# asharakeh/pod_compare

Hardware: AMD Instinct MI355X
Metric: images/sec (BayesOD+MC-dropout, 1280x720) (higher is better)
Workload: dtype f32 (convolutions: every fp32 product from 2-way f16 splits of the power-of-two-scaled fp32 operands, 3 partial products, fp32 accumulate; closer to fp64 than the fp32 MFMA: profiles/r05_f16_split_numerics.txt)

## Files before the change

include/pod_mi355x.h:

```cpp
#ifndef POD_MI355X_H
#define POD_MI355X_H

#include <stddef.h>
#include <stdint.h>

#ifdef __cplusplus
extern "C" {
#endif

#define POD_ABI_VERSION 18
#define POD_MAX_LEVELS 8
#define POD_MAX_CLASSES 16
#define POD_MAX_RUNS 64
#define POD_MAX_TOPK 2048
#define POD_MAX_PROP_SAMPLES 1024
#define POD_MAX_CLS_SAMPLES 64
#define POD_MAX_CANDIDATES 8192
#define POD_MAX_DETECTIONS 128
#define POD_COCO_MAX_IOU 16
#define POD_COCO_MAX_REC 128
#define POD_COCO_MAX_AREA 4
#define POD_COCO_MAX_MAXDET 4
#define POD_COCO_MAX_KEEP 128
#define POD_COCO_LDS_GT 64
// ... 57 lines not shown

int pod_level_topk(const PodConfig* cfg, const PodLevel* levels, uint64_t* cand_keys,
                   int32_t* cand_count, uint64_t* sel_keys, int32_t* sel_count,
                   uint64_t* cat_keys, int32_t* cat_level, int32_t* n_total, pod_stream_t stream);

int pod_gather_candidates(const PodConfig* cfg, const PodLevel* levels, const float* anchors,
                          const uint64_t* cat_keys, const int32_t* cat_level, const int32_t* n_total,
                          int32_t* cand_count, const float* probs_dense,
                          int32_t* cand_anchor_idx, int32_t* cand_level, float* cand_score, int32_t* cand_class,
                          float* cand_probs, float* cand_delta, float* cand_reg_var, float* cand_anchor,
                          float* cand_run_delta ,
                          pod_stream_t stream);

int pod_decode_cov(const PodConfig* cfg, const PodLevel* levels, const int32_t* n_total, int32_t n_capacity,
                   const float* cand_delta, const float* cand_reg_var, const float* cand_anchor,
                   const float* cand_run_delta, const int32_t* cand_anchor_idx, const int32_t* cand_level,
                   const float* eps_prop, int32_t n_replay,
                   float* boxes, float* cov, pod_stream_t stream);

int pod_gather_decode(const PodConfig* cfg, const PodLevel* levels, const float* anchors, const uint64_t* cat_keys,
                      const int32_t* cat_level, const int32_t* n_total, int32_t* cand_count, const float* probs_dense,
                      int32_t* cand_anchor_idx, int32_t* cand_level, float* cand_score,
                      int32_t* cand_class, float* cand_probs, float* cand_delta, float* cand_reg_var, float* cand_anchor,
                      float* cand_run_delta, float* boxes, float* cov, pod_stream_t stream);

size_t pod_nms_scratch_bytes(int32_t n_capacity);
int pod_nms_cluster(const PodConfig* cfg, const int32_t* n_total, int32_t n_capacity,
                    const float* boxes, const float* scores, const int32_t* classes,
                    int32_t* keep, int32_t* n_keep, void* scratch, pod_stream_t stream);

int pod_bayes_fuse(const PodConfig* cfg, const int32_t* n_total, const int32_t* keep, const int32_t* n_keep,
                   const float* boxes, const float* cov, const float* scores, const int32_t* classes,
                   const float* probs, int32_t box_mode, int32_t cls_mode,
                   float* out_boxes, float* out_cov, float* out_scores, int32_t* out_classes, float* out_probs,
                   pod_stream_t stream);

int pod_anchor_stats_merge(const PodConfig* cfg, const int32_t* n_total, const int32_t* keep, const int32_t* n_keep,
                           const float* boxes, const float* cov, const int32_t* classes, const float* probs,
                           float* out_boxes, float* out_cov, float* out_scores, int32_t* out_classes, float* out_probs,
                           pod_stream_t stream);

int pod_ensemble_append(const PodConfig* cfg, const int32_t* keep, const int32_t* n_keep, const float* boxes, const float* cov,
                        const int32_t* classes, const float* probs, int32_t capacity,
                        float* dst_boxes, float* dst_cov, int32_t* dst_classes, float* dst_probs, int32_t* total,
                        pod_stream_t stream);
int pod_ensemble_merge(const PodConfig* cfg, const int32_t* m_total, int32_t capacity, const float* boxes, const float* cov,
                       const int32_t* classes, const float* probs, int32_t* seeds, int32_t* n_seeds,
                       float* out_boxes, float* out_cov, float* out_scores, int32_t* out_classes, float* out_probs,
                       pod_stream_t stream);

int pod_finalize(const PodConfig* cfg, const int32_t* keep, const int32_t* n_rows,
                 const float* boxes, const float* cov, const float* scores, const int32_t* classes,
                 const float* probs, float scale_x, float scale_y, float out_h, float out_w,
                 float* det_boxes, float* det_cov, float* det_scores, int32_t* det_classes, float* det_probs,
                 float* records, int32_t* n_det, pod_stream_t stream);

typedef struct PodDetections {
    float* boxes;  float* cov;  float* scores;  int32_t* classes;  float* probs;  float* records;  int32_t* n_det;
} PodDetections;

int pod_relu_dropout(float* x, int64_t n, float p, uint64_t seed, uint64_t offset, pod_stream_t stream);

int pod_bias_act(float* x, const float* bias, const float* residual, const float* res_bias, int64_t n, int32_t C,
                 int64_t HW, int32_t relu, float p, uint64_t seed, uint64_t offset, pod_stream_t stream);

int pod_bias_act_to_nchw(const float* src, float* dst, const float* bias, int64_t N, int32_t C, int64_t HW, int32_t relu,
                         float p, uint64_t seed, uint64_t offset, pod_stream_t stream);
int pod_bias_act_to_nhwc(const float* src, float* dst, const float* bias, int64_t N, int32_t C, int64_t HW, int32_t relu,
                         pod_stream_t stream);

int pod_expand_dropout(const float* src, float* dst, int64_t n, int32_t copies, float p, uint64_t seed, uint64_t offset,
                       const uint64_t* epoch, pod_stream_t stream);

int pod_wino_filter_transform(const float* weight, float* U, int32_t K, int32_t C, pod_stream_t stream);
int pod_wino_conv3x3(const float* in, float* out, const float* U, const float* bias, const int32_t* blocks, int32_t n_blocks,
                     int32_t C, int32_t K, int32_t k_planes, int32_t relu, float p, uint64_t seed, uint64_t offset,
                     const uint64_t* epoch, pod_stream_t stream);

#define POD_AMAX_SLOTS 16
#define POD_AMAX_STRIDE 32
#define POD_AMAX_FLOATS (POD_AMAX_SLOTS * POD_AMAX_STRIDE)
int pod_absmax(const float* x, int64_t n, float* amax, pod_stream_t stream);

typedef struct PodConvSet {
    const float* in;
    float* out;
    const void* Us;
    const float* bias;
    const float* in_amax;
    float* out_amax;
    uint64_t offset;
    int32_t first_block;
    int32_t replicas;
    int32_t k_planes;
    int32_t reserved;
} PodConvSet;
typedef struct PodWinoConv {
    const int32_t* blocks;
    int32_t n_blocks, n_sets;
    int32_t C, K, relu;
    float p;
    uint64_t seed;
    const uint64_t* epoch;
    int32_t n_splits;
    int32_t reserved;
    int64_t split_stride;
    const int32_t* live_blocks;
    PodConvSet sets[4];
} PodWinoConv;
int64_t pod_wino_filter_split_bytes(int32_t K, int32_t C);
int pod_wino_filter_transform_split(const float* weight, void* Us, int32_t K, int32_t C, pod_stream_t stream);
int pod_wino_conv3x3_split(const PodWinoConv* conv, pod_stream_t stream);

#define POD_SPARSE_LIVE_HEAD 4
#define POD_SPARSE_LIVE_STRIDE 12
int pod_sparse_reach(const PodConfig* cfg, const PodLevel* levels, const uint64_t* cat_keys, const int32_t* cat_level, const int32_t* n_total,
                     uint8_t* reach, uint8_t* scratch, pod_stream_t stream);
int pod_sparse_live_blocks(const PodConfig* cfg, const PodLevel* levels, const int32_t* records, const int32_t* rec_level, int32_t n_records,
                           const uint8_t* reach, int32_t max_reach, int32_t in_reach, int32_t* live, pod_stream_t stream);
int pod_wino_reduce(const float* partials, int32_t n_splits, int64_t split_stride, const float* bias, float* planes, int64_t HW,
                    int32_t K, int32_t k_real, int32_t relu, float* out_amax, pod_stream_t stream);

int pod_stem7x7_filter_split(const float* weight, void* Ws, pod_stream_t stream);
int pod_stem7x7_split(const void* x, int32_t x_is_u8, int32_t H_img, int32_t W_img, const float* mean, const float* stddev, float* y, const void* Ws,
                      const float* bias, int32_t H, int32_t W, int32_t relu, const float* in_amax, float* out_amax, pod_stream_t stream);
int pod_maxpool3x3s2_cl(const float* x, float* y, int32_t H, int32_t W, int32_t C, pod_stream_t stream);
int pod_im2col3x3s2_cl(const float* x, float* y, int32_t H, int32_t W, int32_t C, int32_t relu, pod_stream_t stream);

int pod_match_groundtruth(const float* det_boxes, const float* det_probs, const int32_t* det_off, const int32_t* det_img,
                          int32_t n_det, const float* gt_boxes, const int32_t* gt_off, const int32_t* gt_img, int32_t n_gt,
                          int32_t num_classes, float iou_min, float iou_correct, int32_t* gt_fn, int32_t* gt_match_count,
                          int32_t* gt_match_idx, float* gt_match_iou, int32_t* det_fp, pod_stream_t stream);

int pod_reg_nll(const float* means, const float* covs, const float* gt, int32_t n, float* nll, pod_stream_t stream);

typedef struct PodCocoParams {
    int32_t n_iou, n_rec, n_area, n_maxdet;
    int32_t n_cat;
    int32_t reserved;
    double iou_thrs[POD_COCO_MAX_IOU];
    double rec_thrs[POD_COCO_MAX_REC];
    double area_rng[2 * POD_COCO_MAX_AREA];
    int32_t max_dets[POD_COCO_MAX_MAXDET];
} PodCocoParams;

size_t pod_coco_eval_scratch_bytes(int32_t n_keep, int32_t n_gt);
int pod_coco_eval_images(const PodCocoParams* prm, const int64_t* pairs, int32_t n_pairs, const double* dt_boxes,
                         const double* dt_score, const double* gt_boxes, const double* gt_area, const int32_t* gt_crowd,
                         const int64_t* gt_id, void* scratch, double* kept_score, uint64_t* kept_match, uint64_t* kept_ignore,
                         int32_t* kept_rank, int32_t* npig, pod_stream_t stream);

size_t pod_coco_accumulate_workspace_bytes(int64_t n_kept);
int pod_coco_accumulate(const PodCocoParams* prm, const int64_t* cat_off, int32_t max_seg, int64_t n_kept, const double* kept_score,
                        const uint64_t* kept_match, const uint64_t* kept_ignore, const int32_t* kept_rank, const int32_t* npig,
                        void* workspace, double* precision, double* recall, double* scores, pod_stream_t stream);


int pod_calib_keys(const float* cls_probs, int32_t k1, const float* cov, const int32_t* gt_class, int32_t n_matched, int32_t n,
                   float* cls_entropy, float* reg_entropy, int32_t* det_class, int32_t* class_count, pod_stream_t stream);

int pod_calib_reg_counts(const float* means, const float* cov, const float* gt, const int32_t* det_class, int32_t n_matched,
                         const float* edges, int32_t n_edges, int32_t* counts, pod_stream_t stream);

size_t pod_calib_min_uncertainty_workspace_bytes(int32_t n, int64_t n_pos);
int pod_calib_min_uncertainty(const float* cls_entropy, const float* reg_entropy, const int32_t* det_class, int32_t n, int32_t n_tp,
                              const int32_t* class_off, const int64_t* seg_off, const int32_t* seg_class, int32_t n_seg, int32_t max_seg,
// ... 167 lines not shown
```

pod_compare_amd/csrc/pod_device.h:

```cpp
#pragma once

#include <hip/hip_runtime.h>
#include <stdint.h>

#include <mutex>

#include "../../include/pod_mi355x.h"

#define POD_WAVE 64
#define POD_EPS_MAX 4.9f

#define POD_CHECK_LAUNCH()                                  \
    do {                                                    \
        if (hipGetLastError() != hipSuccess) return POD_E_LAUNCH; \
    } while (0)

template <auto Kernel>
static int pod_lds_opt_in(int bytes) {
    static std::once_flag once[64];
    static hipError_t attr[64];
    int dev = 0;
    if (hipGetDevice(&dev) != hipSuccess || dev < 0 || dev >= 64) return POD_E_LAUNCH;
    std::call_once(once[dev], [dev, bytes] {
        attr[dev] = hipFuncSetAttribute(reinterpret_cast<const void*>(Kernel), hipFuncAttributeMaxDynamicSharedMemorySize, bytes);
    });
    return attr[dev] == hipSuccess ? POD_OK : POD_E_LAUNCH;
}

template <typename... P>
static inline bool pod_aligned(unsigned bytes, const P*... p) {
    return ((... | reinterpret_cast<uintptr_t>(p)) & (bytes - 1u)) == 0;
}
static inline unsigned pod_grid_stride_blocks(int64_t n4, int64_t cap) {
    const int64_t blocks = (n4 + 255) / 256;
    return (unsigned)(blocks < 1 ? 1 : blocks > cap ? cap : blocks);
}

#ifdef POD_TRACE
static __device__ long long g_pod_trace[4096 * 8];
#define POD_STAMP(wg, k)                                                                         \
    do {                                                                                         \
        if ((threadIdx.x & 63) == 0 && threadIdx.x < 64 && (wg) < 4096) g_pod_trace[(wg) * 8 + (k)] = wall_clock64(); \
    } while (0)
#else
#define POD_STAMP(wg, k)
#endif

namespace pod {

struct u32x4 {
    uint32_t x, y, z, w;
};

__device__ __forceinline__ u32x4 philox4x32_10(u32x4 c, uint32_t k0, uint32_t k1) {
    constexpr uint32_t M0 = 0xD2511F53u, M1 = 0xCD9E8D57u, W0 = 0x9E3779B9u, W1 = 0xBB67AE85u;
#pragma unroll
    for (int r = 0; r < 10; ++r) {
        const uint64_t p0 = (uint64_t)M0 * c.x;
        const uint64_t p1 = (uint64_t)M1 * c.z;
        u32x4 n;
        n.x = (uint32_t)(p1 >> 32) ^ c.y ^ k0;
        n.y = (uint32_t)p1;
        n.z = (uint32_t)(p0 >> 32) ^ c.w ^ k1;
        n.w = (uint32_t)p0;
        c = n;
        k0 += W0;
        k1 += W1;
    }
    return c;
}

typedef float f32x4 __attribute__((ext_vector_type(4)));

constexpr uint32_t STREAM_DROPOUT = 0x64726f70u;
#define POD_DROPOUT_THRESH16(p) ((uint32_t)((double)(p) * 65536.0))

__device__ __forceinline__ uint64_t dropout_key(uint64_t seed, const uint64_t* epoch) {
    return epoch ? seed ^ (*epoch * 0x9E3779B97F4A7C15ull) : seed;
}
__device__ __forceinline__ void dropout_words(uint64_t base, uint64_t g, uint32_t c2, uint64_t seed, uint32_t& w0, uint32_t& w1) {
    const uint64_t ctr = base + (g >> 1);
    const u32x4 r = philox4x32_10(u32x4{(uint32_t)ctr, (uint32_t)(ctr >> 32), c2, STREAM_DROPOUT}, (uint32_t)seed, (uint32_t)(seed >> 32));
    w0 = (g & 1) ? r.z : r.x;
    w1 = (g & 1) ? r.w : r.y;
}
template <typename V4>
__device__ __forceinline__ void dropout_mask4(V4& v, uint32_t w0, uint32_t w1, uint32_t thresh, float scale) {
    v.x = (w0 & 0xFFFFu) >= thresh ? v.x * scale : 0.f;
    v.y = (w0 >> 16) >= thresh ? v.y * scale : 0.f;
    v.z = (w1 & 0xFFFFu) >= thresh ? v.z * scale : 0.f;
    v.w = (w1 >> 16) >= thresh ? v.w * scale : 0.f;
}
__device__ __forceinline__ bool dropout_tail_keep(uint64_t base, int64_t n4, uint32_t t, uint64_t seed, uint32_t thresh) {
    const uint64_t ctr = base + (uint64_t)n4 + t;
    const u32x4 r = philox4x32_10(u32x4{(uint32_t)ctr, (uint32_t)(ctr >> 32), 1u, STREAM_DROPOUT}, (uint32_t)seed, (uint32_t)(seed >> 32));
    return (r.x & 0xFFFFu) >= thresh;
}

__device__ __forceinline__ void box_muller16(uint32_t w, float& n0, float& n1) {
    const float u1 = ((float)(w & 0xFFFFu) + 0.5f) * 1.52587890625e-05f;
    const float u2 = ((float)(w >> 16) + 0.5f) * 1.52587890625e-05f;
    const float rad = __builtin_amdgcn_sqrtf(-1.3862943611198906f * __builtin_amdgcn_logf(u1));
    n0 = rad * __builtin_amdgcn_cosf(u2);
    n1 = rad * __builtin_amdgcn_sinf(u2);
}

struct f32x8n {
    float v[8];
};

constexpr uint32_t STREAM_CLS = 0x636c7300u;
constexpr uint32_t STREAM_BOX = 0x626f7800u;

__device__ __forceinline__ f32x8n philox_normals8(uint64_t seed, uint32_t c0, uint32_t c1, uint32_t c2, uint32_t stream) {
    const u32x4 r = philox4x32_10(u32x4{c0, c1, c2, stream}, (uint32_t)seed, (uint32_t)(seed >> 32));
    f32x8n o;
    box_muller16(r.x, o.v[0], o.v[1]);
    box_muller16(r.y, o.v[2], o.v[3]);
    box_muller16(r.z, o.v[4], o.v[5]);
    box_muller16(r.w, o.v[6], o.v[7]);
    return o;
}


__device__ __forceinline__ float sigmoid_ref(float x) { return __fdiv_rn(1.0f, 1.0f + expf(-x)); }
__device__ __forceinline__ float sigmoid_fast(float x) {
    return __builtin_amdgcn_rcpf(1.0f + __builtin_amdgcn_exp2f(-1.4426950408889634f * x));
}

struct Box {
    float x1, y1, x2, y2;
};
#define POD_SCALE_CLAMP 4.135166556742356f

__device__ __forceinline__ Box decode_box(float d0, float d1, float d2, float d3, const Box& a, const float* wts) {
    const float w = a.x2 - a.x1;
    const float h = a.y2 - a.y1;
    const float cx = a.x1 + 0.5f * w;
    const float cy = a.y1 + 0.5f * h;
    const bool unit = wts[0] == 1.0f && wts[1] == 1.0f && wts[2] == 1.0f && wts[3] == 1.0f;
    const float dx = unit ? d0 : __fdiv_rn(d0, wts[0]);
    const float dy = unit ? d1 : __fdiv_rn(d1, wts[1]);
    float dw = unit ? d2 : __fdiv_rn(d2, wts[2]);
    float dh = unit ? d3 : __fdiv_rn(d3, wts[3]);
    dw = fminf(dw, POD_SCALE_CLAMP);
    dh = fminf(dh, POD_SCALE_CLAMP);
// ... 57 lines not shown
```

pod_compare_amd/csrc/pod_wino.h:

```cpp
#pragma once
#include "pod_experiments.h"
#include "pod_split_gemm.h"

namespace pod {

constexpr int WINO_U_FLOATS = 24 * 2 * 64 * 4;
constexpr int WINO_SB_FLOATS = 384 * 32;
constexpr int WINO_LDS_BYTES = 4 * 32 * 4 * 65 * 4;

#ifdef POD_TRACE
static __device__ long long g_wino_trace[8192 * 16];
#define WINO_STAMP(k)                                                                                          \
    do {                                                                                                       \
        if (threadIdx.x == 0 && blockIdx.x < 8192) g_wino_trace[blockIdx.x * 16 + (k)] = __builtin_readcyclecounter(); \
    } while (0)
#define WINO_STAMP_WALL(k)                                                                                     \
    do {                                                                                                       \
        if (threadIdx.x == 0 && blockIdx.x < 8192) g_wino_trace[blockIdx.x * 16 + (k)] = wall_clock64();       \
    } while (0)
#define WINO_STAMP_END()                                                                                       \
    do {                                                                                                       \
        __builtin_amdgcn_s_waitcnt(0);                                                                         \
        WINO_STAMP(5);                                                                                         \
        WINO_STAMP_WALL(13);                                                                                   \
// ... 137 lines not shown
    n += (n + 1) * step <= v ? 1 : 0;
    idx = n;
    return v - n * step;
}

__device__ __forceinline__ void wino_rows(int a, int& row0, int& row1, float& sgn) {
    row0 = a == 0 ? 0 : a == 2 ? 2 : 1;
    row1 = a == 2 ? 1 : a == 3 ? 3 : 2;
    sgn = a == 1 ? 1.0f : -1.0f;
}

__device__ __forceinline__ int* wino_pixel_table(float* lds) { return reinterpret_cast<int*>(lds + 2 * WINO_SB_FLOATS + 2 * 3072); }
#define WINO_FILL_PIXEL_TABLE(pix_tab, B, need, tid)                                                                                  \
    _Pragma("unroll") for (int it_ = 0; it_ < 2; ++it_) {                                                                             \
        const int t = (tid) + 256 * it_;                                                                                              \
        if (t >= 325) break;                                                                                                          \
        const int py = t / 18, px = t - py * 18, vy = (B).y0 - 1 + py, vx = (B).x0 - 1 + px;                                          \
        int m, n;                                                                                                                     \
        const int gy = wino_cell(vy < 0 ? 0 : vy, (B).Hv, (B).rHv, m), gx = wino_cell(vx < 0 ? 0 : vx, (B).Wv, (B).rWv, n), img = m * (B).gcols + n; \
        const bool ok = (t < 324) & (vy >= 0) & (gy < (B).H) & (vx >= 0) & (gx < (B).W) & (n < (B).gcols) & (img < (B).n_img) & ((((need)[it_] >> (t & 31)) & 1u) != 0); \
        (pix_tab)[t] = ok ? img * (B).HWi + gy * (B).W + gx : -1;       \
    }                                                                                                                                 \
    __syncthreads();                                                                                                                  \
    WINO_STAMP(8)

#define WINO_FILL_SLOTS(slot_e, mini_pidx, tid)                                                                                       \
    _Pragma("unroll") for (int i = 0; i < 12; ++i) (slot_e)[i] = g_wino_slots.v[96 * ((tid) >> 6) + 8 * i + (((tid) & 63) >> 3)];     \
    _Pragma("unroll") for (int r = 0; r < 3; ++r) {                                                                                   \
        const int pp = ((((tid) >> 6) * 3 + r) * 64 + ((tid) & 63)) >> 1, py = pp / 21, pi = pp - py * 21, px = 4 * (pi % 5) + pi / 5; \
        (mini_pidx)[r] = py < 18 && pi < 20 && px < 18 ? py * 18 + px : 324;                                                          \
    }
__device__ __forceinline__ int wino_byte_offset(const WinoParams* P, int pix, int part4) {
    return pix >= 0 ? (pix * P->in_stride + part4) * 4 : 0x7FFFFF00;
}
__device__ __forceinline__ void wino_mini_offsets(const WinoParams* P, const int* pix_tab, const int (&mini_pidx)[3], int (&dmini)[3], int lane) {
#pragma unroll
    for (int r = 0; r < 3; ++r) dmini[r] = pix_tab[mini_pidx[r]];
#pragma unroll
    for (int r = 0; r < 3; ++r) dmini[r] = wino_byte_offset(P, dmini[r], 4 * (lane & 1));
}
typedef __attribute__((address_space(3))) void wino_lds_void;
__device__ __forceinline__ void wino_mini_piece(__amdgpu_buffer_rsrc_t rsrc, float* lds, int a, int which, int r, int dmini_r) {
    __builtin_amdgcn_raw_ptr_buffer_load_lds(rsrc, (wino_lds_void*)(lds + 2 * WINO_SB_FLOATS + which * 3072 + (a * 3 + r) * 256), 16, dmini_r, which * 32, 0, 0);
}
__device__ __forceinline__ void wino_patch_piece(__amdgpu_buffer_rsrc_t rsrc, float* stage, int a, int sc, int i, int doff_i) {
    __builtin_amdgcn_raw_ptr_buffer_load_lds(rsrc, (wino_lds_void*)(stage + (a * 12 + i) * 256), 16, doff_i, sc * 128, 0, 0);
}

constexpr int WINO_TS = 260;
constexpr int WINO_ZA = 32 * WINO_TS;
__device__ __forceinline__ bool wino_output_stage(const f32x16 (&acc)[12], float* lds, int a, int i32, int h) {
    if (POD_WINO_ELIM & 128) {
#pragma unroll
        for (int i = 0; i < 12; ++i) asm volatile("" ::"v"(acc[i]));
        return false;
    }
#pragma unroll
    for (int kb = 0; kb < 2; ++kb)
#pragma unroll
        for (int g = 0; g < 4; ++g) {
            f32x4 m[6];
#pragma unroll
            for (int p6 = 0; p6 < 6; ++p6) m[p6] = f32x4{acc[p6 * 2 + kb][4 * g], acc[p6 * 2 + kb][4 * g + 1], acc[p6 * 2 + kb][4 * g + 2], acc[p6 * 2 + kb][4 * g + 3]};
            const f32x4 s1 = m[1] + m[2], d1 = m[1] - m[2], s2 = m[3] + m[4], d2 = m[3] - m[4];
            float* o = lds + (a * 32 + i32) * WINO_TS + kb * 32 + 8 * g + 4 * h;
            *reinterpret_cast<f32x4*>(o) = (m[0] + s1) + s2;
            *reinterpret_cast<f32x4*>(o + 64) = __builtin_elementwise_fma(f32x4{2.f, 2.f, 2.f, 2.f}, d2, d1);
            *reinterpret_cast<f32x4*>(o + 128) = __builtin_elementwise_fma(f32x4{4.f, 4.f, 4.f, 4.f}, s2, s1);
            *reinterpret_cast<f32x4*>(o + 192) = __builtin_elementwise_fma(f32x4{8.f, 8.f, 8.f, 8.f}, d2, d1) + m[5];
        }
    __syncthreads();
    WINO_STAMP(4);
    return !(POD_WINO_ELIM & 32);
}

struct WinoStore {
    float* out;
    const float* bias;
    float* out_amax;
    float inv;
    uint64_t offset;
    int replicas, k_planes;
};
__device__ __forceinline__ void wino_dropout8(f32x4& v0, f32x4& v1, int64_t e, uint64_t offset, uint32_t word, uint64_t key, uint32_t thresh, float scale) {
    const uint64_t ctr = offset + (uint64_t)(e >> 3);
    const u32x4 r4 = philox4x32_10(u32x4{(uint32_t)ctr, (uint32_t)(ctr >> 32), word, STREAM_DROPOUT}, (uint32_t)key, (uint32_t)(key >> 32));
    dropout_mask4(v0, r4.x, r4.y, thresh, scale);
    dropout_mask4(v1, r4.z, r4.w, thresh, scale);
}


template <bool RELU, bool AMAX>
__device__ __forceinline__ float wino_store_planes_form(const WinoBlock& B, const WinoStore& S, const float* lds, int ks) {
    const int tid = threadIdx.x, wave = __builtin_amdgcn_readfirstlane(tid >> 6);
    float lmax = 0.0f;
    const f32x4 inv = f32x4{S.inv, S.inv, S.inv, S.inv};
    const int oy = (tid >> 2) & 15, ox = (tid & 3) * 4, odd = oy & 1;
    const float sg = odd ? -1.0f : 1.0f;
    const int kg0 = ks * 64 + wave;
    const int n_it = (S.k_planes - kg0 + 3) >> 2;
    const float bias_l = S.bias ? S.bias[kg0 + 4 * (tid & 15)] : 0.0f;
    int m;
    const int gy = wino_cell(B.y0 + oy, B.Hv, B.rHv, m);
    int64_t px0[4];
#pragma unroll
    for (int e = 0; e < 4; ++e) {
        int n;
        const int gx = wino_cell(B.x0 + ox + e, B.Wv, B.rWv, n), img = m * B.gcols + n;
        px0[e] = (n < B.gcols && img < B.n_img && gx < B.W && gy < B.H) ? (B.out_px + (int64_t)img * B.HWi) * S.k_planes + (int64_t)gy * B.W + gx : -1;
    }
    const bool vec = px0[0] >= 0 && px0[3] == px0[0] + 3 && (px0[0] & 3) == 0 && (B.HWi & 3) == 0;
    const bool ok[4] = {px0[0] >= 0, px0[1] >= 0, px0[2] >= 0, px0[3] >= 0};
    int64_t q[4];
#pragma unroll
    for (int e = 0; e < 4; ++e) q[e] = (int64_t)kg0 * B.HWi + px0[e];
    const int64_t q_it = (int64_t)4 * B.HWi;
    const int tile = (oy >> 1) * 4 + (tid & 3);
    const float* r = lds + tile * WINO_TS + wave + (odd ? WINO_ZA : 0);
#pragma unroll 1
    for (int it0 = 0; it0 < 16 && it0 < n_it; it0 += 4, r += 16) {
        float z[4][4][3];
        f32x4 v[4];
#pragma unroll
        for (int j = 0; j < 4; ++j)
#pragma unroll
            for (int e = 0; e < 4; ++e)
#pragma unroll
                for (int a = 0; a < 3; ++a) z[j][e][a] = r[4 * j + e * 64 + a * WINO_ZA];
#pragma unroll
        for (int j = 0; j < 4; ++j) {
            const float bias = __builtin_bit_cast(float, __builtin_amdgcn_readlane(__builtin_bit_cast(int, bias_l), it0 + j));
            f32x4 y;
#pragma unroll
            for (int e = 0; e < 4; ++e) y[e] = __builtin_fmaf(sg, z[j][e][2], __builtin_fmaf(sg, z[j][e][1], z[j][e][0]));
            v[j] = __builtin_elementwise_fma(y, inv, f32x4{bias, bias, bias, bias});
            if (RELU) wino_relu4(v[j]);
            if (AMAX) {
                const float mx = wino_absmax4(0.0f, f32x4{ok[0] ? v[j].x : 0.f, ok[1] ? v[j].y : 0.f, ok[2] ? v[j].z : 0.f, ok[3] ? v[j].w : 0.f});
                lmax = fmaxf(lmax, it0 + j < n_it ? mx : 0.0f);
            }
        }
        wino_pin(v[0], v[1], v[2], v[3]);
#pragma unroll
        for (int j = 0; j < 4; ++j) {
            const bool live = it0 + j < n_it;
            if (live && vec) {
                *reinterpret_cast<f32x4*>(S.out + q[0]) = v[j];
            } else if (live) {
                if (ok[0]) S.out[q[0]] = v[j].x;
                if (ok[1]) S.out[q[1]] = v[j].y;
                if (ok[2]) S.out[q[2]] = v[j].z;
                if (ok[3]) S.out[q[3]] = v[j].w;
            }
#pragma unroll
            for (int e = 0; e < 4; ++e) q[e] += q_it;
        }
    }
    return lmax;
}
__device__ __forceinline__ float wino_store_planes(const WinoParams& P, const WinoBlock& B, const WinoStore& S, const float* lds, int ks) {
    switch ((P.relu ? 1 : 0) | (S.out_amax ? 2 : 0)) {
        case 0: return wino_store_planes_form<false, false>(B, S, lds, ks);
        case 1: return wino_store_planes_form<true, false>(B, S, lds, ks);
        case 2: return wino_store_planes_form<false, true>(B, S, lds, ks);
        default: return wino_store_planes_form<true, true>(B, S, lds, ks);
    }
}

template <bool RELU, bool DROP>
__device__ __forceinline__ float wino_store_channels_last_form(const WinoParams& P, const WinoBlock& B, const WinoStore& S, const float* lds, int ks) {
    const int tid = threadIdx.x;
    float lmax = 0.0f;
    const f32x4 inv = f32x4{S.inv, S.inv, S.inv, S.inv};
    const int k8 = (tid & 7) * 8, kg = ks * 64 + k8, ox = (tid >> 3) & 15, odd = tid >> 7;
    const float sg1 = odd ? -1.0f : 1.0f;
    const f32x4 sg = f32x4{sg1, sg1, sg1, sg1};
    f32x4 bias0 = f32x4{0.f, 0.f, 0.f, 0.f}, bias1 = bias0;
    if (S.bias) {
        bias0 = *reinterpret_cast<const f32x4*>(S.bias + kg);
        bias1 = *reinterpret_cast<const f32x4*>(S.bias + kg + 4);
    }
    const uint64_t drop_key = DROP ? dropout_key(P.seed, P.epoch) : 0ull;
    const int n_rep = S.replicas > 0 ? S.replicas : 1;
    const uint32_t word = S.replicas > 0 ? 2u : 0u;
    int n, m;
    const int gx = wino_cell(B.x0 + ox, B.Wv, B.rWv, n);
    const bool col_ok = n < B.gcols && gx < B.W;
    int gy = wino_cell(B.y0 + odd, B.Hv, B.rHv, m);
    int img = m * B.gcols + n;
    const int64_t e_row = (int64_t)(2 * B.W) * P.out_stride, e_wrap = ((int64_t)B.gcols * B.HWi - (int64_t)B.Hv * B.W) * P.out_stride, e_rep = (int64_t)B.HWi * P.out_stride;
    int64_t e = (B.out_px + (int64_t)img * B.HWi + (int64_t)gy * B.W + gx) * P.out_stride + kg - e_row;
    gy -= 2;
    const float* rbase = lds + (ox >> 2) * WINO_TS + (ox & 3) * 64 + k8 + (odd ? WINO_ZA : 0);
#pragma unroll 1
    for (int g = 0; g < 2; ++g) {
        f32x4 z[4][6], v[4][2];
        bool ok[4];
        int64_t er[4];
#pragma unroll
        for (int it = 0; it < 4; ++it) {
            gy += 2;
            const bool wrap = gy >= B.Hv;
            gy -= wrap ? B.Hv : 0;
            img += wrap ? B.gcols : 0;
            e += e_row + (wrap ? e_wrap : 0);
            ok[it] = col_ok && gy < B.H && img < B.n_img;
            er[it] = e;
            const float* r = rbase + (4 * g + it) * 4 * WINO_TS;
            z[it][0] = *reinterpret_cast<const f32x4*>(r); z[it][1] = *reinterpret_cast<const f32x4*>(r + 4);
            z[it][2] = *reinterpret_cast<const f32x4*>(r + WINO_ZA); z[it][3] = *reinterpret_cast<const f32x4*>(r + WINO_ZA + 4);
            z[it][4] = *reinterpret_cast<const f32x4*>(r + 2 * WINO_ZA); z[it][5] = *reinterpret_cast<const f32x4*>(r + 2 * WINO_ZA + 4);
        }
#pragma unroll
        for (int it = 0; it < 4; ++it) {
            v[it][0] = __builtin_elementwise_fma(__builtin_elementwise_fma(sg, z[it][4], __builtin_elementwise_fma(sg, z[it][2], z[it][0])), inv, bias0);
            v[it][1] = __builtin_elementwise_fma(__builtin_elementwise_fma(sg, z[it][5], __builtin_elementwise_fma(sg, z[it][3], z[it][1])), inv, bias1);
            if (RELU) {
                wino_relu4(v[it][0]);
                wino_relu4(v[it][1]);
            }
            const float mx = wino_absmax4(wino_absmax4(0.0f, v[it][0]), v[it][1]);
            lmax = fmaxf(lmax, ok[it] ? (DROP ? mx * P.scale : mx) : 0.0f);
        }
#pragma unroll 1
        for (int rep = 0; rep < n_rep; ++rep) {
            f32x4 w[4][2];
#pragma unroll
            for (int it = 0; it < 4; ++it) {
                w[it][0] = v[it][0];
                w[it][1] = v[it][1];
                if (DROP && !(POD_WINO_ELIM & 64)) wino_dropout8(w[it][0], w[it][1], er[it], S.offset, word, drop_key, P.thresh, P.scale);
            }
#pragma unroll
            for (int it = 0; it < 4; ++it) wino_pin(w[it][0], w[it][1]);
#pragma unroll
            for (int it = 0; it < 4; ++it) {
                if (ok[it]) {
                    *reinterpret_cast<f32x4*>(S.out + er[it]) = w[it][0];
                    *reinterpret_cast<f32x4*>(S.out + er[it] + 4) = w[it][1];
                }
                er[it] += e_rep;
            }
        }
    }
    return lmax;
}
__device__ __forceinline__ float wino_store_channels_last(const WinoParams& P, const WinoBlock& B, const WinoStore& S, const float* lds, int ks) {
    switch ((P.relu ? 1 : 0) | (P.thresh ? 2 : 0)) {
        case 0: return wino_store_channels_last_form<false, false>(P, B, S, lds, ks);
        case 1: return wino_store_channels_last_form<true, false>(P, B, S, lds, ks);
        case 2: return wino_store_channels_last_form<false, true>(P, B, S, lds, ks);
        default: return wino_store_channels_last_form<true, true>(P, B, S, lds, ks);
    }
}

}
```

Before: 143.2.

## Use buffer stores with out-of-range predication in Winograd output epilogues

The Winograd store epilogues now write through raw buffer stores with 32-bit byte offsets. Masked lanes get bit 31 set in their offset so the hardware range check drops the write, which replaces per-lane branches and 64-bit address arithmetic. Layouts whose output range is too large for a 32-bit offset fall back to new 'far' paths that keep 64-bit indexing. Philox also uses a three-input XOR bitop builtin where the compiler provides one. The changes add code size and depend on the buffer resource range being computed correctly.

```diff
diff --git a/include/pod_mi355x.h b/include/pod_mi355x.h
--- a/include/pod_mi355x.h
+++ b/include/pod_mi355x.h
@@ -163,6 +163,7 @@
 #define POD_AMAX_FLOATS (POD_AMAX_SLOTS * POD_AMAX_STRIDE)
 int pod_absmax(const float* x, int64_t n, float* amax, pod_stream_t stream);
 
+#define POD_WINO_STORE_RANGE_MAX 0x7FFFFF00LL
 typedef struct PodConvSet {
     const float* in;
     float* out;
diff --git a/pod_compare_amd/csrc/pod_device.h b/pod_compare_amd/csrc/pod_device.h
--- a/pod_compare_amd/csrc/pod_device.h
+++ b/pod_compare_amd/csrc/pod_device.h
@@ -52,6 +52,14 @@
     uint32_t x, y, z, w;
 };
 
+__device__ __forceinline__ uint32_t xor3(uint32_t a, uint32_t b, uint32_t c) {
+#if __has_builtin(__builtin_amdgcn_bitop3_b32)
+    return __builtin_amdgcn_bitop3_b32(a, b, c, 0x96);
+#else
+    return a ^ b ^ c;
+#endif
+}
+
 __device__ __forceinline__ u32x4 philox4x32_10(u32x4 c, uint32_t k0, uint32_t k1) {
     constexpr uint32_t M0 = 0xD2511F53u, M1 = 0xCD9E8D57u, W0 = 0x9E3779B9u, W1 = 0xBB67AE85u;
 #pragma unroll
@@ -59,9 +67,9 @@
         const uint64_t p0 = (uint64_t)M0 * c.x;
         const uint64_t p1 = (uint64_t)M1 * c.z;
         u32x4 n;
-        n.x = (uint32_t)(p1 >> 32) ^ c.y ^ k0;
+        n.x = xor3((uint32_t)(p1 >> 32), c.y, k0);
         n.y = (uint32_t)p1;
-        n.z = (uint32_t)(p0 >> 32) ^ c.w ^ k1;
+        n.z = xor3((uint32_t)(p0 >> 32), c.w, k1);
         n.w = (uint32_t)p0;
         c = n;
         k0 += W0;
diff --git a/pod_compare_amd/csrc/pod_wino.h b/pod_compare_amd/csrc/pod_wino.h
--- a/pod_compare_amd/csrc/pod_wino.h
+++ b/pod_compare_amd/csrc/pod_wino.h
@@ -243,41 +243,73 @@
     uint64_t offset;
     int replicas, k_planes;
 };
-__device__ __forceinline__ void wino_dropout8(f32x4& v0, f32x4& v1, int64_t e, uint64_t offset, uint32_t word, uint64_t key, uint32_t thresh, float scale) {
-    const uint64_t ctr = offset + (uint64_t)(e >> 3);
+__device__ __forceinline__ void wino_dropout8(f32x4& v0, f32x4& v1, uint64_t ctr, uint32_t word, uint64_t key, uint32_t thresh, float scale) {
     const u32x4 r4 = philox4x32_10(u32x4{(uint32_t)ctr, (uint32_t)(ctr >> 32), word, STREAM_DROPOUT}, (uint32_t)key, (uint32_t)(key >> 32));
     dropout_mask4(v0, r4.x, r4.y, thresh, scale);
     dropout_mask4(v1, r4.z, r4.w, thresh, scale);
 }
 
+constexpr uint32_t WINO_STORE_DROP = 0x80000000u;
+static_assert(POD_WINO_STORE_RANGE_MAX < WINO_STORE_DROP, "bit 31 of an offset must lie past every resource");
+__device__ __forceinline__ void wino_buffer_store4(__amdgpu_buffer_rsrc_t rsrc, uint32_t byte_off, f32x4 v) {
+    __builtin_amdgcn_raw_buffer_store_b128(__builtin_bit_cast(sg_u32x4, v), rsrc, (int)byte_off, 0, 0);
+}
+__device__ __forceinline__ void wino_buffer_store1(__amdgpu_buffer_rsrc_t rsrc, uint32_t byte_off, float v) {
+    __builtin_amdgcn_raw_buffer_store_b32(__builtin_bit_cast(uint32_t, v), rsrc, (int)byte_off, 0, 0);
+}
+
+struct WinoPlanesThread {
+    int wave, kg0, n_it;
+    float sg;
+    bool ok[4];
+    int img[4], pix[4];
+    const float* r;
+};
+__device__ __forceinline__ WinoPlanesThread wino_planes_thread(const WinoBlock& B, const WinoStore& S, const float* lds, int ks) {
+    WinoPlanesThread T;
+    const int tid = threadIdx.x;
+    T.wave = __builtin_amdgcn_readfirstlane(tid >> 6);
+    const int oy = (tid >> 2) & 15, ox = (tid & 3) * 4, odd = oy & 1;
+    T.sg = odd ? -1.0f : 1.0f;
+    T.kg0 = ks * 64 + T.wave;
+    T.n_it = (S.k_planes - T.kg0 + 3) >> 2;
+    int m;
+    const int gy = wino_cell(B.y0 + oy, B.Hv, B.rHv, m);
+#pragma unroll
+    for (int e = 0; e < 4; ++e) {
+        int n;
+        const int gx = wino_cell(B.x0 + ox + e, B.Wv, B.rWv, n);
+        T.img[e] = m * B.gcols + n;
+        T.pix[e] = gy * B.W + gx;
+        T.ok[e] = n < B.gcols && T.img[e] < B.n_img && gx < B.W && gy < B.H;
+    }
+    T.r = lds + ((oy >> 1) * 4 + (tid & 3)) * WINO_TS + T.wave + (odd ? WINO_ZA : 0);
+    return T;
+}
+__device__ __forceinline__ f32x4 wino_planes_values(const float (&z)[4][3], float sg, f32x4 inv, float bias) {
+    f32x4 y;
+#pragma unroll
+    for (int e = 0; e < 4; ++e) y[e] = __builtin_fmaf(sg, z[e][2], __builtin_fmaf(sg, z[e][1], z[e][0]));
+    return __builtin_elementwise_fma(y, inv, f32x4{bias, bias, bias, bias});
+}
 
 template <bool RELU, bool AMAX>
-__device__ __forceinline__ float wino_store_planes_form(const WinoBlock& B, const WinoStore& S, const float* lds, int ks) {
-    const int tid = threadIdx.x, wave = __builtin_amdgcn_readfirstlane(tid >> 6);
+__device__ __forceinline__ float wino_store_planes_form(const WinoBlock& B, const WinoStore& S, __amdgpu_buffer_rsrc_t rsrc, const float* lds, int ks) {
+    const WinoPlanesThread T = wino_planes_thread(B, S, lds, ks);
+    const int tid = threadIdx.x, n_it = T.n_it;
     float lmax = 0.0f;
     const f32x4 inv = f32x4{S.inv, S.inv, S.inv, S.inv};
-    const int oy = (tid >> 2) & 15, ox = (tid & 3) * 4, odd = oy & 1;
-    const float sg = odd ? -1.0f : 1.0f;
-    const int kg0 = ks * 64 + wave;
-    const int n_it = (S.k_planes - kg0 + 3) >> 2;
-    const float bias_l = S.bias ? S.bias[kg0 + 4 * (tid & 15)] : 0.0f;
-    int m;
-    const int gy = wino_cell(B.y0 + oy, B.Hv, B.rHv, m);
-    int64_t px0[4];
-#pragma unroll
-    for (int e = 0; e < 4; ++e) {
-        int n;
-        const int gx = wino_cell(B.x0 + ox + e, B.Wv, B.rWv, n), img = m * B.gcols + n;
-        px0[e] = (n < B.gcols && img < B.n_img && gx < B.W && gy < B.H) ? (B.out_px + (int64_t)img * B.HWi) * S.k_planes + (int64_t)gy * B.W + gx : -1;
-    }
-    const bool vec = px0[0] >= 0 && px0[3] == px0[0] + 3 && (px0[0] & 3) == 0 && (B.HWi & 3) == 0;
-    const bool ok[4] = {px0[0] >= 0, px0[1] >= 0, px0[2] >= 0, px0[3] >= 0};
-    int64_t q[4];
-#pragma unroll
-    for (int e = 0; e < 4; ++e) q[e] = (int64_t)kg0 * B.HWi + px0[e];
-    const int64_t q_it = (int64_t)4 * B.HWi;
-    const int tile = (oy >> 1) * 4 + (tid & 3);
-    const float* r = lds + tile * WINO_TS + wave + (odd ? WINO_ZA : 0);
+    const float sg = T.sg;
+    const float bias_l = S.bias ? S.bias[T.kg0 + 4 * (tid & 15)] : 0.0f;
+    const bool ok[4] = {T.ok[0], T.ok[1], T.ok[2], T.ok[3]};
+    uint32_t q[4];
+#pragma unroll
+    for (int e = 0; e < 4; ++e) q[e] = 4u * ((uint32_t)(T.img[e] * S.k_planes + T.kg0) * (uint32_t)B.HWi + (uint32_t)T.pix[e]);
+    const uint32_t q_it = 16u * (uint32_t)B.HWi;
+    const bool vec = ok[0] && ok[3] && q[3] == q[0] + 12 && (((uint32_t)B.out_px * (uint32_t)S.k_planes + (q[0] >> 2)) & 3) == 0 && (B.HWi & 3) == 0;
+    const bool sc[4] = {!vec && ok[0], !vec && ok[1], !vec && ok[2], !vec && ok[3]};
+    const bool any_sc = __builtin_amdgcn_ballot_w64(sc[0] || sc[1] || sc[2] || sc[3]) != 0;
+    const float* r = T.r;
 #pragma unroll 1
     for (int it0 = 0; it0 < 16 && it0 < n_it; it0 += 4, r += 16) {
         float z[4][4][3];
@@ -291,10 +323,7 @@
 #pragma unroll
         for (int j = 0; j < 4; ++j) {
             const float bias = __builtin_bit_cast(float, __builtin_amdgcn_readlane(__builtin_bit_cast(int, bias_l), it0 + j));
-            f32x4 y;
-#pragma unroll
-            for (int e = 0; e < 4; ++e) y[e] = __builtin_fmaf(sg, z[j][e][2], __builtin_fmaf(sg, z[j][e][1], z[j][e][0]));
-            v[j] = __builtin_elementwise_fma(y, inv, f32x4{bias, bias, bias, bias});
+            v[j] = wino_planes_values(z[j], sg, inv, bias);
             if (RELU) wino_relu4(v[j]);
             if (AMAX) {
                 const float mx = wino_absmax4(0.0f, f32x4{ok[0] ? v[j].x : 0.f, ok[1] ? v[j].y : 0.f, ok[2] ? v[j].z : 0.f, ok[3] ? v[j].w : 0.f});
@@ -303,79 +332,131 @@
         }
         wino_pin(v[0], v[1], v[2], v[3]);
 #pragma unroll
-        for (int j = 0; j < 4; ++j) {
-            const bool live = it0 + j < n_it;
-            if (live && vec) {
-                *reinterpret_cast<f32x4*>(S.out + q[0]) = v[j];
-            } else if (live) {
-                if (ok[0]) S.out[q[0]] = v[j].x;
-                if (ok[1]) S.out[q[1]] = v[j].y;
-                if (ok[2]) S.out[q[2]] = v[j].z;
-                if (ok[3]) S.out[q[3]] = v[j].w;
-            }
-#pragma unroll
-            for (int e = 0; e < 4; ++e) q[e] += q_it;
-        }
+        for (int j = 0; j < 4; ++j) wino_buffer_store4(rsrc, (vec ? q[0] + j * q_it : WINO_STORE_DROP) | (it0 + j < n_it ? 0u : WINO_STORE_DROP), v[j]);
+        if (any_sc) {
+#pragma unroll
+            for (int j = 0; j < 4; ++j)
+#pragma unroll
+                for (int e = 0; e < 4; ++e)
+                    wino_buffer_store1(rsrc, (sc[e] ? q[e] + j * q_it : WINO_STORE_DROP) | (it0 + j < n_it ? 0u : WINO_STORE_DROP), v[j][e]);
+        }
+#pragma unroll
+        for (int e = 0; e < 4; ++e) q[e] += 4 * q_it;
     }
     return lmax;
 }
-__device__ __forceinline__ float wino_store_planes(const WinoParams& P, const WinoBlock& B, const WinoStore& S, const float* lds, int ks) {
-    switch ((P.relu ? 1 : 0) | (S.out_amax ? 2 : 0)) {
-        case 0: return wino_store_planes_form<false, false>(B, S, lds, ks);
-        case 1: return wino_store_planes_form<true, false>(B, S, lds, ks);
-        case 2: return wino_store_planes_form<false, true>(B, S, lds, ks);
-        default: return wino_store_planes_form<true, true>(B, S, lds, ks);
-    }
-}
-
-template <bool RELU, bool DROP>
-__device__ __forceinline__ float wino_store_channels_last_form(const WinoParams& P, const WinoBlock& B, const WinoStore& S, const float* lds, int ks) {
-    const int tid = threadIdx.x;
+__device__ __forceinline__ float wino_store_planes_far(const WinoParams& P, const WinoBlock& B, const WinoStore& S, const float* lds, int ks) {
+    const WinoPlanesThread T = wino_planes_thread(B, S, lds, ks);
     float lmax = 0.0f;
     const f32x4 inv = f32x4{S.inv, S.inv, S.inv, S.inv};
-    const int k8 = (tid & 7) * 8, kg = ks * 64 + k8, ox = (tid >> 3) & 15, odd = tid >> 7;
-    const float sg1 = odd ? -1.0f : 1.0f;
-    const f32x4 sg = f32x4{sg1, sg1, sg1, sg1};
-    f32x4 bias0 = f32x4{0.f, 0.f, 0.f, 0.f}, bias1 = bias0;
+    int64_t q[4];
+#pragma unroll
+    for (int e = 0; e < 4; ++e) q[e] = ((B.out_px + (int64_t)T.img[e] * B.HWi) * S.k_planes + (int64_t)T.kg0 * B.HWi + T.pix[e]);
+    const bool vec = T.ok[0] && T.ok[3] && q[3] == q[0] + 3 && (q[0] & 3) == 0 && (B.HWi & 3) == 0;
+    const float* r = T.r;
+#pragma unroll 1
+    for (int it = 0; it < 16 && it < T.n_it; ++it, r += 4) {
+        float z[4][3];
+#pragma unroll
+        for (int e = 0; e < 4; ++e)
+#pragma unroll
+            for (int a = 0; a < 3; ++a) z[e][a] = r[e * 64 + a * WINO_ZA];
+        f32x4 v = wino_planes_values(z, T.sg, inv, S.bias ? S.bias[T.kg0 + 4 * it] : 0.0f);
+        if (P.relu) wino_relu4(v);
+        if (vec) *reinterpret_cast<f32x4*>(S.out + q[0]) = v;
+#pragma unroll
+        for (int e = 0; e < 4; ++e) {
+            if (T.ok[e]) lmax = fmaxf(lmax, fabsf(v[e]));
+            if (T.ok[e] && !vec) S.out[q[e]] = v[e];
+            q[e] += (int64_t)4 * B.HWi;
+        }
+    }
+    return lmax;
+}
+__device__ __forceinline__ float wino_store_planes(const WinoParams& P, const WinoBlock& B, const WinoStore& S, const float* lds, int ks) {
+    const int64_t range = (int64_t)B.n_img * B.HWi * S.k_planes * 4;
+    if (range > POD_WINO_STORE_RANGE_MAX) return wino_store_planes_far(P, B, S, lds, ks);
+    const auto rsrc = __builtin_amdgcn_make_buffer_rsrc(S.out + B.out_px * S.k_planes, 0, (int)range, 0x00020000);
+    switch ((P.relu ? 1 : 0) | (S.out_amax ? 2 : 0)) {
+        case 0: return wino_store_planes_form<false, false>(B, S, rsrc, lds, ks);
+        case 1: return wino_store_planes_form<true, false>(B, S, rsrc, lds, ks);
+        case 2: return wino_store_planes_form<false, true>(B, S, rsrc, lds, ks);
+        default: return wino_store_planes_form<true, true>(B, S, rsrc, lds, ks);
+    }
+}
+
+struct WinoRowsThread {
+    int k8, kg, img, gy;
+    bool col_ok;
+    int64_t px;
+    float sg;
+    f32x4 bias0, bias1;
+    const float* rbase;
+};
+__device__ __forceinline__ WinoRowsThread wino_rows_thread(const WinoBlock& B, const WinoStore& S, const float* lds, int ks) {
+    WinoRowsThread T;
+    const int tid = threadIdx.x, ox = (tid >> 3) & 15, odd = tid >> 7;
+    T.k8 = (tid & 7) * 8;
+    T.kg = ks * 64 + T.k8;
+    T.sg = odd ? -1.0f : 1.0f;
+    T.bias0 = f32x4{0.f, 0.f, 0.f, 0.f};
+    T.bias1 = T.bias0;
     if (S.bias) {
-        bias0 = *reinterpret_cast<const f32x4*>(S.bias + kg);
-        bias1 = *reinterpret_cast<const f32x4*>(S.bias + kg + 4);
-    }
+        T.bias0 = *reinterpret_cast<const f32x4*>(S.bias + T.kg);
+        T.bias1 = *reinterpret_cast<const f32x4*>(S.bias + T.kg + 4);
+    }
+    int n, m;
+    const int gx = wino_cell(B.x0 + ox, B.Wv, B.rWv, n);
+    T.col_ok = n < B.gcols && gx < B.W;
+    T.gy = wino_cell(B.y0 + odd, B.Hv, B.rHv, m);
+    T.img = m * B.gcols + n;
+    T.px = (int64_t)T.gy * B.W + gx;
+    T.rbase = lds + (ox >> 2) * WINO_TS + (ox & 3) * 64 + T.k8 + (odd ? WINO_ZA : 0);
+    return T;
+}
+__device__ __forceinline__ void wino_rows_values(const f32x4 (&z)[6], f32x4 sg, f32x4 inv, f32x4 bias0, f32x4 bias1, f32x4& v0, f32x4& v1) {
+    v0 = __builtin_elementwise_fma(__builtin_elementwise_fma(sg, z[4], __builtin_elementwise_fma(sg, z[2], z[0])), inv, bias0);
+    v1 = __builtin_elementwise_fma(__builtin_elementwise_fma(sg, z[5], __builtin_elementwise_fma(sg, z[3], z[1])), inv, bias1);
+}
+__device__ __forceinline__ void wino_rows_read(const float* r, f32x4 (&z)[6]) {
+    z[0] = *reinterpret_cast<const f32x4*>(r); z[1] = *reinterpret_cast<const f32x4*>(r + 4);
+    z[2] = *reinterpret_cast<const f32x4*>(r + WINO_ZA); z[3] = *reinterpret_cast<const f32x4*>(r + WINO_ZA + 4);
+    z[4] = *reinterpret_cast<const f32x4*>(r + 2 * WINO_ZA); z[5] = *reinterpret_cast<const f32x4*>(r + 2 * WINO_ZA + 4);
+}
+
+template <bool RELU, bool DROP>
+__device__ __forceinline__ float wino_store_channels_last_form(const WinoParams& P, const WinoBlock& B, const WinoStore& S, __amdgpu_buffer_rsrc_t rsrc, const float* lds, int ks) {
+    const WinoRowsThread T = wino_rows_thread(B, S, lds, ks);
+    float lmax = 0.0f;
+    const f32x4 inv = f32x4{S.inv, S.inv, S.inv, S.inv}, sg = f32x4{T.sg, T.sg, T.sg, T.sg};
     const uint64_t drop_key = DROP ? dropout_key(P.seed, P.epoch) : 0ull;
     const int n_rep = S.replicas > 0 ? S.replicas : 1;
     const uint32_t word = S.replicas > 0 ? 2u : 0u;
-    int n, m;
-    const int gx = wino_cell(B.x0 + ox, B.Wv, B.rWv, n);
-    const bool col_ok = n < B.gcols && gx < B.W;
-    int gy = wino_cell(B.y0 + odd, B.Hv, B.rHv, m);
-    int img = m * B.gcols + n;
-    const int64_t e_row = (int64_t)(2 * B.W) * P.out_stride, e_wrap = ((int64_t)B.gcols * B.HWi - (int64_t)B.Hv * B.W) * P.out_stride, e_rep = (int64_t)B.HWi * P.out_stride;
-    int64_t e = (B.out_px + (int64_t)img * B.HWi + (int64_t)gy * B.W + gx) * P.out_stride + kg - e_row;
-    gy -= 2;
-    const float* rbase = lds + (ox >> 2) * WINO_TS + (ox & 3) * 64 + k8 + (odd ? WINO_ZA : 0);
+    const uint32_t e_row = 8u * (uint32_t)B.W * (uint32_t)P.out_stride, e_rep = 4u * (uint32_t)B.HWi * (uint32_t)P.out_stride;
+    const uint32_t e_wrap = 4u * ((uint32_t)B.gcols * (uint32_t)B.HWi - (uint32_t)B.Hv * (uint32_t)B.W) * (uint32_t)P.out_stride;
+    const uint64_t ctr0 = S.offset + ((uint64_t)(B.out_px * P.out_stride) >> 3);
+    int gy = T.gy - 2, img = T.img;
+    uint32_t e = 4u * (((uint32_t)img * (uint32_t)B.HWi + (uint32_t)T.px) * (uint32_t)P.out_stride + (uint32_t)T.kg) - e_row;
 #pragma unroll 1
     for (int g = 0; g < 2; ++g) {
         f32x4 z[4][6], v[4][2];
         bool ok[4];
-        int64_t er[4];
+        uint32_t er[4], step[4];
 #pragma unroll
         for (int it = 0; it < 4; ++it) {
             gy += 2;
             const bool wrap = gy >= B.Hv;
             gy -= wrap ? B.Hv : 0;
             img += wrap ? B.gcols : 0;
-            e += e_row + (wrap ? e_wrap : 0);
-            ok[it] = col_ok && gy < B.H && img < B.n_img;
-            er[it] = e;
-            const float* r = rbase + (4 * g + it) * 4 * WINO_TS;
-            z[it][0] = *reinterpret_cast<const f32x4*>(r); z[it][1] = *reinterpret_cast<const f32x4*>(r + 4);
-            z[it][2] = *reinterpret_cast<const f32x4*>(r + WINO_ZA); z[it][3] = *reinterpret_cast<const f32x4*>(r + WINO_ZA + 4);
-            z[it][4] = *reinterpret_cast<const f32x4*>(r + 2 * WINO_ZA); z[it][5] = *reinterpret_cast<const f32x4*>(r + 2 * WINO_ZA + 4);
+            e += e_row + (wrap ? e_wrap : 0u);
+            ok[it] = T.col_ok && gy < B.H && img < B.n_img;
+            er[it] = ok[it] ? e : WINO_STORE_DROP;
+            step[it] = ok[it] ? e_rep : 0u;
+            wino_rows_read(T.rbase + (4 * g + it) * 4 * WINO_TS, z[it]);
         }
 #pragma unroll
         for (int it = 0; it < 4; ++it) {
-            v[it][0] = __builtin_elementwise_fma(__builtin_elementwise_fma(sg, z[it][4], __builtin_elementwise_fma(sg, z[it][2], z[it][0])), inv, bias0);
-            v[it][1] = __builtin_elementwise_fma(__builtin_elementwise_fma(sg, z[it][5], __builtin_elementwise_fma(sg, z[it][3], z[it][1])), inv, bias1);
+            wino_rows_values(z[it], sg, inv, T.bias0, T.bias1, v[it][0], v[it][1]);
             if (RELU) {
                 wino_relu4(v[it][0]);
                 wino_relu4(v[it][1]);
@@ -390,29 +471,69 @@
             for (int it = 0; it < 4; ++it) {
                 w[it][0] = v[it][0];
                 w[it][1] = v[it][1];
-                if (DROP && !(POD_WINO_ELIM & 64)) wino_dropout8(w[it][0], w[it][1], er[it], S.offset, word, drop_key, P.thresh, P.scale);
+                if (DROP && !(POD_WINO_ELIM & 64)) wino_dropout8(w[it][0], w[it][1], ctr0 + (er[it] >> 5), word, drop_key, P.thresh, P.scale);
             }
 #pragma unroll
             for (int it = 0; it < 4; ++it) wino_pin(w[it][0], w[it][1]);
 #pragma unroll
             for (int it = 0; it < 4; ++it) {
-                if (ok[it]) {
-                    *reinterpret_cast<f32x4*>(S.out + er[it]) = w[it][0];
-                    *reinterpret_cast<f32x4*>(S.out + er[it] + 4) = w[it][1];
-                }
-                er[it] += e_rep;
+                wino_buffer_store4(rsrc, er[it], w[it][0]);
+                wino_buffer_store4(rsrc, er[it] + 16, w[it][1]);
+                er[it] += step[it];
             }
         }
     }
     return lmax;
 }
+__device__ __forceinline__ float wino_store_channels_last_far(const WinoParams& P, const WinoBlock& B, const WinoStore& S, const float* lds, int ks) {
+    const WinoRowsThread T = wino_rows_thread(B, S, lds, ks);
+    float lmax = 0.0f;
+    const f32x4 inv = f32x4{S.inv, S.inv, S.inv, S.inv}, sg = f32x4{T.sg, T.sg, T.sg, T.sg};
+    const bool drop = P.thresh != 0;
+    const uint64_t drop_key = drop ? dropout_key(P.seed, P.epoch) : 0ull;
+    const int n_rep = S.replicas > 0 ? S.replicas : 1;
+    const uint32_t word = S.replicas > 0 ? 2u : 0u;
+    const int64_t e_row = (int64_t)(2 * B.W) * P.out_stride, e_wrap = ((int64_t)B.gcols * B.HWi - (int64_t)B.Hv * B.W) * P.out_stride, e_rep = (int64_t)B.HWi * P.out_stride;
+    int gy = T.gy - 2, img = T.img;
+    int64_t e = (B.out_px + (int64_t)img * B.HWi + T.px) * P.out_stride + T.kg - e_row;
+#pragma unroll 1
+    for (int i = 0; i < 8; ++i) {
+        gy += 2;
+        const bool wrap = gy >= B.Hv;
+        gy -= wrap ? B.Hv : 0;
+        img += wrap ? B.gcols : 0;
+        e += e_row + (wrap ? e_wrap : 0);
+        if (!(T.col_ok && gy < B.H && img < B.n_img)) continue;
+        f32x4 z[6], v0, v1;
+        wino_rows_read(T.rbase + i * 4 * WINO_TS, z);
+        wino_rows_values(z, sg, inv, T.bias0, T.bias1, v0, v1);
+        if (P.relu) {
+            wino_relu4(v0);
+            wino_relu4(v1);
+        }
+        const float mx = wino_absmax4(wino_absmax4(0.0f, v0), v1);
+        lmax = fmaxf(lmax, drop ? mx * P.scale : mx);
+#pragma unroll 1
+        for (int rep = 0; rep < n_rep; ++rep) {
+            f32x4 w0 = v0, w1 = v1;
+            const int64_t er = e + rep * e_rep;
+            if (drop) wino_dropout8(w0, w1, S.offset + (uint64_t)(er >> 3), word, drop_key, P.thresh, P.scale);
+            *reinterpret_cast<f32x4*>(S.out + er) = w0;
+            *reinterpret_cast<f32x4*>(S.out + er + 4) = w1;
+        }
+    }
+    return lmax;
+}
 __device__ __forceinline__ float wino_store_channels_last(const WinoParams& P, const WinoBlock& B, const WinoStore& S, const float* lds, int ks) {
+    const int64_t range = (int64_t)(B.n_img + (S.replicas > 0 ? S.replicas - 1 : 0)) * B.HWi * P.out_stride * 4;
+    if (range > POD_WINO_STORE_RANGE_MAX) return wino_store_channels_last_far(P, B, S, lds, ks);
+    const auto rsrc = __builtin_amdgcn_make_buffer_rsrc(S.out + B.out_px * P.out_stride, 0, (int)range, 0x00020000);
     switch ((P.relu ? 1 : 0) | (P.thresh ? 2 : 0)) {
-        case 0: return wino_store_channels_last_form<false, false>(P, B, S, lds, ks);
-        case 1: return wino_store_channels_last_form<true, false>(P, B, S, lds, ks);
-        case 2: return wino_store_channels_last_form<false, true>(P, B, S, lds, ks);
-        default: return wino_store_channels_last_form<true, true>(P, B, S, lds, ks);
-    }
-}
-
-}
+        case 0: return wino_store_channels_last_form<false, false>(P, B, S, rsrc, lds, ks);
+        case 1: return wino_store_channels_last_form<true, false>(P, B, S, rsrc, lds, ks);
+        case 2: return wino_store_channels_last_form<false, true>(P, B, S, rsrc, lds, ks);
+        default: return wino_store_channels_last_form<true, true>(P, B, S, rsrc, lds, ks);
+    }
+}
+
+}
```

Result: no change. 144.5 (median of 6 runs) (+1.0%).
